# facebookresearch/FlowDec

Measured on AMD Instinct MI355X. Metric: 48 kHz audio-seconds/sec (RTF) for FlowDec-75m @ 6 ODE steps, higher is better.
Workload: dtype bf16; 1 GPU; flowdec_75m enhance(): global batch=8 x 2 s clips @48 kHz (8 per GPU), 6-step euler (NFE 6), T_pad=256 frames, inputs resident in HBM, initial noise drawn inside the timed call, output waveforms all-gathered; global_batch=8, nfe=6, parallelism=batch-shard x1, hipgraph=True, conv_algo=auto

## Files before the change

flowdec_amd/csrc/conv_wino4.hip:

```cpp
#include <type_traits>

#include "conv_common.h"

namespace {

using namespace fdconv;

typedef _Float16 f16;
typedef __attribute__((ext_vector_type(2))) _Float16 f16x2;
typedef __attribute__((ext_vector_type(8))) _Float16 f16x8;
typedef unsigned int u32x2 __attribute__((ext_vector_type(2)));
typedef float f32x2 __attribute__((ext_vector_type(2)));

constexpr int cmax(int a, int b) { return a > b ? a : b; }

constexpr int NTH = 512, TH = 16, TW = 16, HH = TH + 2, HW = TW + 2, BN = 256;
constexpr int CK = 16;
constexpr int SLAB = BN * 32;
constexpr int RSLOT = 2048, NRING = 6;
static_assert(18 % NRING == 0, "the two-chunk loop body turns the ring a whole number of times");
constexpr int RING_BYTES = 8 * NRING * RSLOT;
constexpr int VXI = HH * 4 * 32;
constexpr int V_BYTES = 6 * VXI;
constexpr int V_OFF = RING_BYTES;
constexpr int AFF_OFF = V_OFF + 2 * V_BYTES;
constexpr int RAW_OFF = AFF_OFF + AFF_BYTES;
constexpr int RROW = 20;
constexpr int RROW_BYTES = RROW * 64;
constexpr int RAW_PASSES = 3;
constexpr int RAW_BYTES = RAW_PASSES * NTH * 16;
constexpr int MAIN_BYTES = RAW_OFF + RAW_BYTES;
constexpr int X_BYTES = 8 * 8192;
constexpr int S_PITCH = 128 * 4 + 16;
constexpr int S_BYTES = 128 * S_PITCH;
constexpr int SK_OFF = S_BYTES, SK_BYTES = 4 * NTH * 16;
constexpr int SCK = 2, SCD = 3;
constexpr int WS_BYTES = SCK * SLAB;
constexpr int XS_OFF = SCD * WS_BYTES, XS_BYTES = SCK * 8192;
constexpr int BIAS_OFF = 2 * S_BYTES;
static_assert(BIAS_OFF >= 2 * X_BYTES && BIAS_OFF >= SK_OFF + 2 * SK_BYTES && XS_OFF + SCD * XS_BYTES <= 160 * 1024, "epilogue LDS map");
constexpr int ISC_OFF = BIAS_OFF + 1024;
constexpr int STAT_OFF = ISC_OFF + 1024;
constexpr int LDS_BYTES = cmax(MAIN_BYTES, STAT_OFF + 16384);
constexpr int NPIECE = HH * RROW * 4;
static_assert(LDS_BYTES <= 160 * 1024 && NPIECE <= RAW_PASSES * NTH && AFF_BYTES <= 4 * 1024 && RAW_OFF % 128 == 0, "LDS layout");
constexpr int raw_slot(int c) { return c < 16 ? c + (c >> 2) : (c == 16 ? 14 : 19); }
constexpr int raw_flip(int c) { return c < 16 ? (c >> 3) & 1 : 0; }
constexpr int U_EXP = 9;
constexpr float RAW_MAX = 6000.f;

__device__ __forceinline__ unsigned pack_f16(float a, float b) {
  f16x2 r = {(f16)a, (f16)b};
  return __builtin_bit_cast(unsigned, r);
}
__device__ __forceinline__ f16x2 h2(unsigned u) { return __builtin_bit_cast(f16x2, u); }
__device__ __forceinline__ unsigned u2(f16x2 v) { return __builtin_bit_cast(unsigned, v); }

__device__ __forceinline__ void glds16s(const void* sbase, unsigned voff, unsigned lds_dst) {
  asm volatile("s_mov_b32 m0, %2\n\ts_nop 0\n\tglobal_load_lds_dwordx4 %0, %1" ::"v"(voff), "s"(sbase), "s"(lds_dst) : "memory");
}
__device__ __forceinline__ void glds16s_x2(const void* sbase, unsigned voff, unsigned lds_dst) {
  asm volatile("s_mov_b32 m0, %2\n\ts_nop 0\n\tglobal_load_lds_dwordx4 %0, %1\n\tglobal_load_lds_dwordx4 %0, %1 offset:1024" ::"v"(voff), "s"(sbase), "s"(lds_dst)
               : "memory");
}

template <bool ACT, bool SKIP, bool SC>
__global__ __launch_bounds__(NTH, 2) void conv_wino4_kernel(ConvArgs p) {
  static_assert(!(SKIP && SC), "residual input and folded shortcut exclude each other in this kernel");
  extern __shared__ __attribute__((aligned(16))) char smem[];
  FD_T2(const unsigned long long t2_entry = __builtin_amdgcn_s_memtime();)

  const int bid = blockIdx.x, nblk = gridDim.x;
  int lid;
  {
    const int xcd = bid & 7, qq = nblk >> 3, rr = nblk & 7;
    lid = (xcd < rr ? xcd * (qq + 1) : rr * (qq + 1) + (xcd - rr) * qq) + (bid >> 3);
  }
  if (p.reversed) lid = nblk - 1 - lid;
  int pt = lid;
  const int tw_i = pt % p.tiles_w; pt /= p.tiles_w;
  const int th_i = pt % p.tiles_h;
  const int b = pt / p.tiles_h;
  const int h0 = th_i * TH, w0 = tw_i * TW;
  const int H = p.H, W = p.W;

  const int t = threadIdx.x;
  const int lane = t & 63;
  const int wave = __builtin_amdgcn_readfirstlane(t >> 6);
  const int cq = wave & 3, xt = wave >> 2;

  auto opaque = [&](int v) { asm volatile("" : "+v"(v)); return v; };
  const size_t img_elems = (size_t)H * W;
  const int hb = h0 > 0 ? h0 - 1 : 0;
  const size_t band_pix = (size_t)b * img_elems + (size_t)hb * W;
  const bf16* const sb0 = reinterpret_cast<const bf16*>(p.seg[0].src) + band_pix * p.seg[0].C;
  const bool two3 = p.nseg > 1 && p.seg[1].taps == 9;
  const bf16* const sb1 = two3 ? reinterpret_cast<const bf16*>(p.seg[1].src) + band_pix * p.seg[1].C : sb0;
  const int sC0 = p.seg[0].C, sC1 = two3 ? p.seg[1].C : 0;
  const int nch0 = sC0 / CK, n3 = nch0 + sC1 / CK;
  int hpix[RAW_PASSES];
#pragma unroll
  for (int i = 0; i < RAW_PASSES; ++i) {
    const int sl = t + i * NTH;
    const int slot = sl >> 2;
    const int hr = slot / RROW, ps = slot - hr * RROW;
    const int hc = (ps == 4 || ps == 9 || hr >= HH) ? -1 : ps == 14 ? 16 : ps == 19 ? 17 : ps - ps / 5;
    const int gh = h0 - 1 + hr, gw = w0 - 1 + hc;
    const bool ok = hc >= 0 && gh >= 0 && gh < H && gw >= 0 && gw < W;
    hpix[i] = ((ok ? (gh - hb) * W + gw : 0) << 2) | ((sl & 3) ^ (ok ? 2 * raw_flip(hc) : 0));
  }
  int pA, pB, vbits;
  {
    const int hrow = t >> 5, wt = (t >> 3) & 3, word = t & 7;
    auto raw_at = [&](int c) { return hrow * RROW_BYTES + raw_slot(c) * 64 + raw_flip(c) * 32 + word * 4; };
    const int tidx = hrow * 4 + wt;
    const int vrel = tidx * 32 + (((word >> 2) ^ ((tidx >> 3) & 1)) * 16) + (word & 3) * 4;
    pA = raw_at(4 * wt) | (vrel << 16);
    pB = raw_at(4 * wt + 4) | (raw_at(4 * wt + 5) << 16);
    const int gh = h0 - 1 + hrow, ghe = gh + 14;
    vbits = (w0 - 1 + 4 * wt >= 0 ? 1 : 0) | (gh >= 0 && gh < H ? 2 : 0) | (w0 + 4 * wt + 4 < W ? 4 : 0) | (ghe >= 0 && ghe < H ? 8 : 0);
  }
  const bf16* nbase = sb0;
  int nC2 = 0, ncb = 0;
  int cnext = 0;
  auto next_chunk = [&]() {
    if (cnext < n3) {
      const bool first = cnext < nch0;
      const int cch = first ? cnext : cnext - nch0;
      nbase = first ? sb0 : sb1;
      nC2 = (first ? sC0 : sC1) * 2;
      ncb = cch * CK * 2;
    }
    ++cnext;
  };
  const unsigned rawdst = (unsigned)(RAW_OFF + wave * 1024);
  auto load_halo = [&]() {
    const int on = cnext <= n3 ? 1 : 0;
#pragma unroll
    for (int i = 0; i < RAW_PASSES; ++i) {
      const int hp = opaque(hpix[i]);
      glds16s(nbase, (unsigned)(((hp >> 2) * nC2 + ncb + (hp & 3) * 16) * on), rawdst + i * 8192);
    }
  };
  int affa = AFF_OFF + (t & 7) * 16;
  auto load_affine = [&]() {
    if constexpr (ACT) {
      if (wave < AFF_BYTES / 1024) {
        const int o = opaque(t) * 16;
        glds16s(p.affine + (size_t)b * p.affC * 2, (unsigned)(o < n3 * CK * 8 ? o : 0), (unsigned)(AFF_OFF + wave * 1024));
      }
    }
  };

  auto produce = [&](const bool extra, const int e, const int vbuf, const int affo) {
    const int pa = opaque(pA), pb = opaque(pB), vbt = opaque(vbits);
    const char* const rp = smem + RAW_OFF + (extra ? 14 * RROW_BYTES : 0);
    const int a0 = (pa & 0xffff) ^ (e << 5), a4 = (pb & 0xffff) ^ (e << 5), a5 = (int)((unsigned)pb >> 16) ^ (e << 5);
    const int vrel = (int)((unsigned)pa >> 16);
    char* const vb = smem + V_OFF + vbuf * V_BYTES + (extra ? (vrel ^ 16) + 14 * 4 * 32 : vrel);
    unsigned w_[6];
#pragma unroll
    for (int j = 0; j < 4; ++j) w_[j] = *reinterpret_cast<const unsigned*>(rp + a0 + j * 64);
    w_[4] = *reinterpret_cast<const unsigned*>(rp + a4);
    w_[5] = *reinterpret_cast<const unsigned*>(rp + a5);
    f32x4 af = {0.f, 0.f, 0.f, 0.f};
    if constexpr (ACT) af = *reinterpret_cast<const f32x4*>(smem + opaque(affa) + affo);
    const unsigned mrow = (unsigned)((int)((unsigned)vbt << (extra ? 28 : 30)) >> 31);
    const unsigned m0 = mrow & (unsigned)((int)((unsigned)vbt << 31) >> 31), m5 = mrow & (unsigned)((int)((unsigned)vbt << 29) >> 31);
#pragma unroll
    for (int j = 0; j < 6; ++j) {
      const unsigned u = w_[j];
      const float x0 = __builtin_bit_cast(float, u << 16), x1 = __builtin_bit_cast(float, u & 0xffff0000u);
      unsigned r;
      if constexpr (ACT) {
        const f16x2 zc = {(f16)RAW_MAX, (f16)RAW_MAX};
        r = u2(__builtin_elementwise_min(h2(pack_f16(fd_silu(fmaf(x0, af[0], af[1])), fd_silu(fmaf(x1, af[2], af[3])))), zc));
      } else
        r = pack_f16(__builtin_amdgcn_fmed3f(x0, -RAW_MAX, RAW_MAX), __builtin_amdgcn_fmed3f(x1, -RAW_MAX, RAW_MAX));
      w_[j] = r & (j == 0 ? m0 : j == 5 ? m5 : mrow);
    }
    const f16x2 c4 = {(f16)4.f, (f16)4.f}, cm4 = {(f16)-4.f, (f16)-4.f}, cm5 = {(f16)-5.f, (f16)-5.f}, c2 = {(f16)2.f, (f16)2.f},
                cm2 = {(f16)-2.f, (f16)-2.f};
    const f16x2 z0 = h2(w_[0]), z1 = h2(w_[1]), z2 = h2(w_[2]), z3 = h2(w_[3]), z4 = h2(w_[4]), z5 = h2(w_[5]);
    const f16x2 t1 = __builtin_elementwise_fma(z2, cm4, z4);
    const f16x2 t2 = __builtin_elementwise_fma(z1, cm4, z3);
    const f16x2 t3 = z4 - z2, t4 = z3 - z1;
    *reinterpret_cast<unsigned*>(vb + 0 * VXI) = u2(__builtin_elementwise_fma(z0, c4, __builtin_elementwise_fma(z2, cm5, z4)));
    *reinterpret_cast<unsigned*>(vb + 1 * VXI) = u2(t1 + t2);
    *reinterpret_cast<unsigned*>(vb + 2 * VXI) = u2(t1 - t2);
    *reinterpret_cast<unsigned*>(vb + 4 * VXI) = u2(__builtin_elementwise_fma(t4, c2, t3));
    *reinterpret_cast<unsigned*>(vb + 5 * VXI) = u2(__builtin_elementwise_fma(t4, cm2, t3));
    *reinterpret_cast<unsigned*>(vb + 3 * VXI) = u2(__builtin_elementwise_fma(z1, c4, __builtin_elementwise_fma(z3, cm5, z5)));
  };
  const bool extra_wave = wave == 1;

  const char* wp = reinterpret_cast<const char*>(p.w) + (size_t)xt * 9 * SLAB + cq * 2048;
  asm volatile("" : "+s"(wp));
  const unsigned lane16 = (unsigned)(lane * 16);
  const unsigned wring = (unsigned)(wave * NRING * RSLOT);
  auto dma_step = [&](int f, int slot) {
    glds16s_x2(wp + (f / 9) * 18 * SLAB + (f % 9) * SLAB, lane16, wring + slot * RSLOT);
  };

  const int l31 = lane & 31, lh = lane >> 5;
  const int wa_lane = (int)wring + l31 * 32 + ((lh ^ ((l31 >> 3) & 1)) * 16);
  const int vb0 = V_OFF + xt * 3 * VXI  + l31 * 32 + ((lh ^ ((l31 >> 3) & 1)) * 16);
  const int vb1 = (vb0 ^ ((l31 & 4) << 2)) + 128;

  f32x16 acc[3][2][2];
#pragma unroll
  for (int x = 0; x < 3; ++x)
#pragma unroll
    for (int ct = 0; ct < 2; ++ct)
#pragma unroll
      for (int nt = 0; nt < 2; ++nt)
#pragma unroll
        for (int e = 0; e < 16; ++e) acc[x][ct][nt][e] = 0.f;

  auto lds_wait = [&]() { asm volatile("s_waitcnt lgkmcnt(0)" ::: "memory"); };
  auto barrier = [&]() {
    __builtin_amdgcn_s_barrier();
    asm volatile("" ::: "memory");
  };

  u32x4 qa[3], qb[3];
  auto mma = [&](int xl, int ct, int nt, const u32x4& a, const u32x4& bq) {
    acc[xl][ct][nt] = __builtin_amdgcn_mfma_f32_32x32x16_f16(__builtin_bit_cast(f16x8, a), __builtin_bit_cast(f16x8, bq), acc[xl][ct][nt], 0, 0, 0);
  };
  auto rd = [&](int off) { return *reinterpret_cast<const u32x4*>(smem + off); };
  auto a_off = [&](int k18, int ct) { return wa_lane + (k18 % NRING) * RSLOT + ct * 1024; };
  auto b_off = [&](int k18, int nt) {
    const int s = k18 % 9, half = (k18 / 9) & 1;
    const int dy = s % 3;
    return (dy == 0 ? vb0 : dy == 1 ? vb1 : (vb0 ^ 16) + 256) + half * V_BYTES + (s / 3) * VXI + nt * 1024;
  };

  next_chunk();
  load_halo();
  load_affine();
#pragma unroll
  for (int k = 0; k < NRING; ++k) dma_step(k, k);
  asm volatile("s_waitcnt vmcnt(0)" ::: "memory");
  barrier();
  produce(false, 0, 0, 0);
  if (extra_wave) produce(true, 0, 0, 0);
  next_chunk();
  lds_wait();
  barrier();
  FD_T2(const unsigned long long t2_first = __builtin_amdgcn_s_memtime();)
  qa[0] = rd(a_off(0, 0)); qb[0] = rd(b_off(0, 0)); qb[1] = rd(b_off(0, 1)); qa[1] = rd(a_off(0, 1));

  constexpr int NW = 2 * (NRING - 2);
  for (int c = 0; c < n3; c += 2) {
    int xg = xt;
    asm volatile("" : "+s"(xg));
#pragma clang loop unroll(full)
    for (int k = 0; k < 18; ++k) {
      const int s = k % 9, half = k / 9;
      const int vn = half ^ 1;
      const int xl = s / 3;
      u32x4 &A0 = qa[(2 * k) % 3], &A1 = qa[(2 * k + 1) % 3], &A2 = qa[(2 * k + 2) % 3];
      u32x4 &B0 = qb[(2 * k) % 3], &B1 = qb[(2 * k + 1) % 3], &B2 = qb[(2 * k + 2) % 3];
      if (s >= 4 && s <= 7 && half == 0) asm volatile("s_waitcnt vmcnt(%0)" ::"n"(NW + RAW_PASSES) : "memory");
      else asm volatile("s_waitcnt vmcnt(%0)" ::"n"(NW) : "memory");
      if (s == 8 || (s == 3 && half == 0)) { lds_wait(); barrier(); }
      A2 = rd(a_off(k + 1, 0));
      B2 = rd(b_off(k + 1, 0));
      __builtin_amdgcn_sched_barrier(0);
      mma(xl, 0, 0, A0, B0);
      mma(xl, 0, 1, A0, B1);
      __builtin_amdgcn_sched_barrier(0);
      A0 = rd(a_off(k + 1, 1));
      mma(xl, 1, 0, A1, B0);
      __builtin_amdgcn_sched_barrier(0);
      B0 = rd(b_off(k + 1, 1));
      if (s == 3) { next_chunk(); if (half == 0) load_halo(); }
      dma_step(k + NRING, k % NRING);
      mma(xl, 1, 1, A1, B1);
      __builtin_amdgcn_sched_barrier(0);
      if (s == 0) { if (xg == 0) produce(false, half ^ 1, vn, 128 * (1 + half)); }
      if (s == 1) { if (xg == 1) produce(false, half ^ 1, vn, 128 * (1 + half)); }
      if (s == 2) { if (extra_wave) produce(true, half ^ 1, vn, 128 * (1 + half)); }
      __builtin_amdgcn_sched_barrier(0);
    }
    wp += 36 * SLAB;
    asm volatile("" : "+s"(wp));
    affa += 2 * CK * 8;
  }
  asm volatile("s_waitcnt vmcnt(0)" ::: "memory");
  __syncthreads();
  FD_T2(const unsigned long long t2_loop = __builtin_amdgcn_s_memtime();)

  const size_t row0_pix = (size_t)b * img_elems + (size_t)h0 * W;
  bf16* const out = reinterpret_cast<bf16*>(p.out) + row0_pix * p.Cout;
  const bf16* const skip = SKIP ? reinterpret_cast<const bf16*>(p.skip) + row0_pix * p.Cout : nullptr;
  float* const biast = reinterpret_cast<float*>(smem + BIAS_OFF);
  float* const statt = reinterpret_cast<float*>(smem + STAT_OFF);
  float* const isct = reinterpret_cast<float*>(smem + ISC_OFF);
  auto load_bias_table = [&]() {
    if (t < BN) {
      biast[t] = p.bias ? p.bias[(size_t)(p.bias_rows > 1 ? b : 0) * p.Cout + t] * p.scale : 0.f;
      isct[t] = p.w_scale[t] * p.scale;
    }
  };
  if constexpr (!SC) load_bias_table();
  auto out_off = [&](int tt, int ct, int nt, int ps) {
    const int oct = tt & 15, pp = tt >> 4;
    const int rh = nt * 8 + (pp >> 2), gw = w0 + 4 * (pp & 3) + ps;
    return (rh * W + gw) * p.Cout + ct * 128 + oct * 8;
  };
  auto skip_dma = [&](int r) {
    if constexpr (SKIP) {
      const int tt = opaque(t);
#pragma unroll
      for (int ps = 0; ps < 4; ++ps)
        glds16s(skip, (unsigned)(out_off(tt, r >> 1, r & 1, ps) * 2), (unsigned)(SK_OFF + (r & 1) * SK_BYTES + ps * NTH * 16 + wave * 1024));
    }
  };
  skip_dma(0);
  skip_dma(1);
  FD_T2(
  unsigned long long t2_r[5] = {0, 0, 0, 0, 0};
  t2_r[0] = __builtin_amdgcn_s_memtime();
  )

  const float ka = xt ? 0.f : 1.f, ks = xt ? 4.f : 1.f, kb = xt ? 1.f : 0.f, kd = xt ? 8.f : 1.f, kq = xt ? 0.25f : 1.f;
  auto e1_round = [&](int rd_, int xoff) {
    const int ct = rd_ >> 1, nt = rd_ & 1;
    f32x16 &m0 = acc[0][ct][nt], &m1 = acc[1][ct][nt], &m2 = acc[2][ct][nt];
    const f32x2 kd2 = {kd, kd}, kq2 = {kq, kq}, ka2 = {ka, ka}, ks2 = {ks, ks}, kb2 = {kb, kb};
    char* const xmine = smem + xoff + wave * 8192 + lane * 16;
    const char* const xpeer = smem + xoff + (wave ^ 4) * 8192 + lane * 16;
#pragma unroll
    for (int g = 0; g < 4; ++g) {
      f32x2 snd[2];
#pragma unroll
      for (int h = 0; h < 2; ++h) {
        const int e = 4 * g + 2 * h;
        const f32x2 a1 = {m1[e], m1[e + 1]}, a2 = {m2[e], m2[e + 1]};
        const f32x2 s_ = a1 + a2, d_ = (a1 - a2) * kd2;
        m2[e] = s_[0]; m2[e + 1] = s_[1];
        m1[e] = d_[0]; m1[e + 1] = d_[1];
        snd[h] = d_ * kq2;
      }
      *reinterpret_cast<f32x4*>(xmine + g * 1024) = f32x4{m2[4 * g], m2[4 * g + 1], m2[4 * g + 2], m2[4 * g + 3]};
      *reinterpret_cast<f32x4*>(xmine + 4096 + g * 1024) = f32x4{snd[0][0], snd[0][1], snd[1][0], snd[1][1]};
    }
    lds_wait();
    barrier();
#pragma unroll
    for (int g = 0; g < 4; ++g) {
      const f32x4 r0 = *reinterpret_cast<const f32x4*>(xpeer + g * 1024), r1 = *reinterpret_cast<const f32x4*>(xpeer + 4096 + g * 1024);
#pragma unroll
      for (int h = 0; h < 2; ++h) {
        const int e = 4 * g + 2 * h;
        const f32x2 mm = {m0[e], m0[e + 1]}, ss = {m2[e], m2[e + 1]}, dd = {m1[e], m1[e + 1]};
        const f32x2 q0 = {r0[2 * h], r0[2 * h + 1]}, q1 = {r1[2 * h], r1[2 * h + 1]};
        const f32x2 ya = __builtin_elementwise_fma(ka2, mm, __builtin_elementwise_fma(ks2, ss, q0));
        const f32x2 yb = __builtin_elementwise_fma(kb2, mm, dd + q1);
        m0[e] = ya[0]; m0[e + 1] = ya[1];
        m1[e] = yb[0]; m1[e + 1] = yb[1];
      }
    }
  };
  float ssum[8], ssq[8];
  auto e3_round = [&](int rd_, int soff) {
    const int ct = rd_ >> 1, nt = rd_ & 1;
    f32x16 &m0 = acc[0][ct][nt], &m1 = acc[1][ct][nt];
    char* const sbuf = smem + soff;
    if (nt == 0) {
#pragma unroll
      for (int j = 0; j < 8; ++j) ssum[j] = ssq[j] = 0.f;
    }
    {
      char* const sbase = sbuf + ((2 * xt) * 32 + l31) * S_PITCH + (cq * 32 + 4 * lh) * 4;
#pragma unroll
      for (int g = 0; g < 4; ++g) {
        *reinterpret_cast<f32x4*>(sbase + g * 32) = f32x4{m0[4 * g], m0[4 * g + 1], m0[4 * g + 2], m0[4 * g + 3]};
        *reinterpret_cast<f32x4*>(sbase + 32 * S_PITCH + g * 32) = f32x4{m1[4 * g], m1[4 * g + 1], m1[4 * g + 2], m1[4 * g + 3]};
      }
    }
    lds_wait();
    barrier();
    __builtin_amdgcn_sched_barrier(0);
    if constexpr (SKIP) {
      if (rd_ == 0 || rd_ == 3) asm volatile("s_waitcnt vmcnt(4)" ::: "memory");
      else asm volatile("s_waitcnt vmcnt(8)" ::: "memory");
    }
    {
      const int tt = opaque(t);
      const int oct = tt & 15, pp = tt >> 4;
      const f32x4 bA = *reinterpret_cast<const f32x4*>(biast + ct * 128 + oct * 8), bB = *reinterpret_cast<const f32x4*>(biast + ct * 128 + oct * 8 + 4);
      const float bv[8] = {bA[0], bA[1], bA[2], bA[3], bB[0], bB[1], bB[2], bB[3]};
      const f32x4 iA = *reinterpret_cast<const f32x4*>(isct + ct * 128 + oct * 8), iB = *reinterpret_cast<const f32x4*>(isct + ct * 128 + oct * 8 + 4);
      const float iv[8] = {iA[0], iA[1], iA[2], iA[3], iB[0], iB[1], iB[2], iB[3]};
#pragma unroll
      for (int bt = 0; bt < 2; ++bt) {
        u32x4 packed[2];
        int ooff[2];
#pragma unroll
        for (int q = 0; q < 2; ++q) {
          const int ps = 2 * bt + q;
          ooff[q] = out_off(tt, ct, nt, ps);
          const float* sp = reinterpret_cast<const float*>(sbuf + (pp + ps * 32) * S_PITCH) + oct * 8;
          const f32x4 v0 = *reinterpret_cast<const f32x4*>(sp), v1 = *reinterpret_cast<const f32x4*>(sp + 4);
          float v[8] = {v0[0], v0[1], v0[2], v0[3], v1[0], v1[1], v1[2], v1[3]};
          if constexpr (SKIP) {
            const u32x4 skr = *reinterpret_cast<const u32x4*>(smem + SK_OFF + (rd_ & 1) * SK_BYTES + (ps * NTH + tt) * 16);
            const bf16x8 sk = __builtin_bit_cast(bf16x8, skr);
#pragma unroll
            for (int k = 0; k < 4; ++k) {
              const f32x2 s2_ = {(float)sk[2 * k], (float)sk[2 * k + 1]}, sc2 = {p.scale, p.scale}, b2 = {bv[2 * k], bv[2 * k + 1]};
              const f32x2 i2 = {iv[2 * k], iv[2 * k + 1]}, x_ = {v[2 * k], v[2 * k + 1]};
              const f32x2 r_ = __builtin_elementwise_fma(x_, i2, __builtin_elementwise_fma(s2_, sc2, b2));
              v[2 * k] = r_[0]; v[2 * k + 1] = r_[1];
            }
          }
#pragma unroll
          for (int k = 0; k < 4; ++k) {
#pragma clang fp contract(off)
            f32x2 x = {v[2 * k], v[2 * k + 1]};
            f32x2 s1 = {ssum[2 * k], ssum[2 * k + 1]}, s2 = {ssq[2 * k], ssq[2 * k + 1]};
            if constexpr (!SKIP) {
              const f32x2 b2 = {bv[2 * k], bv[2 * k + 1]}, i2 = {iv[2 * k], iv[2 * k + 1]};
              x = __builtin_elementwise_fma(x, i2, b2);
            }
            s1 += x;
            s2 = __builtin_elementwise_fma(x, x, s2);
            v[2 * k] = x[0]; v[2 * k + 1] = x[1];
            ssum[2 * k] = s1[0]; ssum[2 * k + 1] = s1[1];
            ssq[2 * k] = s2[0]; ssq[2 * k + 1] = s2[1];
          }
          bf16x8 tv;
#pragma unroll
          for (int j = 0; j < 8; ++j) tv[j] = (bf16)v[j];
          packed[q] = __builtin_bit_cast(u32x4, tv);
        }
#pragma unroll
        for (int q = 0; q < 2; ++q) *reinterpret_cast<u32x4*>(out + ooff[q]) = packed[q];
      }
    }
    if (nt == 1 && p.stats) {
#pragma unroll
      for (int j = 0; j < 8; ++j) {
        ssum[j] += __shfl_xor(ssum[j], 16, 64); ssq[j] += __shfl_xor(ssq[j], 16, 64);
        ssum[j] += __shfl_xor(ssum[j], 32, 64); ssq[j] += __shfl_xor(ssq[j], 32, 64);
      }
      if (lane < 16) {
        float* rec = statt + ((ct * 8 + wave) * 16 + lane) * 16;
#pragma unroll
        for (int j = 0; j < 4; ++j) *reinterpret_cast<f32x4*>(rec + 4 * j) = f32x4{ssum[2 * j], ssq[2 * j], ssum[2 * j + 1], ssq[2 * j + 1]};
      }
    }
  };

  if constexpr (SC) {
#pragma unroll
    for (int rd_ = 0; rd_ < 4; ++rd_) {
      e1_round(rd_, (rd_ & 1) * X_BYTES);
      __builtin_amdgcn_sched_barrier(0);
    }
    lds_wait();
    barrier();
    FD_T2(t2_r[1] = __builtin_amdgcn_s_memtime();)
    {
      const int nsc = p.nseg - (sC1 ? 2 : 1);
      const Seg q0 = p.seg[p.nseg - nsc], q1 = p.seg[p.nseg - 1];
      const int S0 = q0.C, Stot = S0 + (nsc > 1 ? q1.C : 0);
      const int nstage = Stot / (16 * SCK);
      const bf16* const xb0 = reinterpret_cast<const bf16*>(q0.src) + row0_pix * q0.C;
      const bf16* const xb1 = reinterpret_cast<const bf16*>(q1.src) + row0_pix * q1.C;
      const char* const wsc = reinterpret_cast<const char*>(p.w) + (size_t)(n3 + 1) * 18 * SLAB + cq * 2048;
      static_assert(SCK == 2, "a stage row = 2 K steps x 2 halves x 16 B; K step kk of the weights is loaded by wave group xt = kk");
      int xsrc[2];
#pragma unroll
      for (int i = 0; i < 2; ++i) {
        const int r = ((i * 8 + wave) * 64 + lane) >> 2;
        const int xtile = r & 63, xj = r >> 6;
        const int piece = (lane & 3) ^ ((r >> 2) & 3);
        xsrc[i] = (((xtile >> 2) * W + w0 + 4 * (xtile & 3) + xj) << 8) | (piece * 16);
      }
      const unsigned lane16e = (unsigned)(lane * 16);
      auto stage_dma = [&](int st, int slot) {
        const int ste = st < nstage ? st : 0;
        const int c0 = ste * 16 * SCK;
        const bool first = c0 < S0;
        const bf16* const xb = first ? xb0 : xb1;
        const int Cs = first ? S0 : Stot - S0, cc = first ? c0 : c0 - S0;
#pragma unroll
        for (int i = 0; i < 2; ++i)
          glds16s(xb, (unsigned)(((xsrc[i] >> 8) * Cs + cc) * 2 + (xsrc[i] & 255)), (unsigned)(XS_OFF + slot * XS_BYTES + i * 8192 + wave * 1024));
        glds16s_x2(wsc + (size_t)(ste * SCK + xt) * SLAB, lane16e, (unsigned)(slot * WS_BYTES + xt * SLAB + cq * 2048));
      };
      const int wa_sc = cq * 2048 + l31 * 32 + ((lh ^ ((l31 >> 3) & 1)) * 16);
      const int xb_row = XS_OFF + ((2 * xt) * 64 + l31) * 64;
      const int xb_sw = (l31 >> 2) & 3;
#pragma unroll
      for (int d = 0; d < SCD - 1; ++d) stage_dma(d, d);
      int slot = 0;
      for (int st = 0; st < nstage; ++st) {
        asm volatile("s_waitcnt vmcnt(%0)" ::"n"(4 * (SCD - 2)) : "memory");
        lds_wait();
        barrier();
        const int nslot = slot == 0 ? SCD - 1 : slot - 1;
        stage_dma(st + SCD - 1, nslot);
        const int wo = slot * WS_BYTES, xo = slot * XS_BYTES;
        u32x4 af[SCK][2], bq[SCK][2][2];
#pragma unroll
        for (int kk = 0; kk < SCK; ++kk) {
          af[kk][0] = rd(wa_sc + wo + kk * SLAB);
          af[kk][1] = rd(wa_sc + wo + kk * SLAB + 1024);
#pragma unroll
          for (int pl = 0; pl < 2; ++pl)
#pragma unroll
            for (int nt = 0; nt < 2; ++nt) bq[kk][pl][nt] = rd(xb_row + xo + (pl * 64 + nt * 32) * 64 + (((kk * 2 + lh) ^ xb_sw) * 16));
        }
        __builtin_amdgcn_sched_barrier(0);
#pragma unroll
        for (int kk = 0; kk < SCK; ++kk)
#pragma unroll
          for (int pl = 0; pl < 2; ++pl)
#pragma unroll
            for (int nt = 0; nt < 2; ++nt) {
              acc[pl][0][nt] = __builtin_amdgcn_mfma_f32_32x32x16_bf16(__builtin_bit_cast(bf16x8, af[kk][0]), __builtin_bit_cast(bf16x8, bq[kk][pl][nt]), acc[pl][0][nt], 0, 0, 0);
              acc[pl][1][nt] = __builtin_amdgcn_mfma_f32_32x32x16_bf16(__builtin_bit_cast(bf16x8, af[kk][1]), __builtin_bit_cast(bf16x8, bq[kk][pl][nt]), acc[pl][1][nt], 0, 0, 0);
            }
        __builtin_amdgcn_sched_barrier(0);
        slot = slot + 1 == SCD ? 0 : slot + 1;
      }
      asm volatile("s_waitcnt vmcnt(0)" ::: "memory");
      lds_wait();
      barrier();
      load_bias_table();
    }
    FD_T2(t2_r[2] = __builtin_amdgcn_s_memtime();)
#pragma unroll
    for (int rd_ = 0; rd_ < 4; ++rd_) {
      e3_round(rd_, (rd_ & 1) * S_BYTES);
      __builtin_amdgcn_sched_barrier(0);
    }
  } else {
#pragma unroll
    for (int rd_ = 0; rd_ < 4; ++rd_) {
      e1_round(rd_, 0);
      if constexpr (SKIP) { lds_wait(); barrier(); }
      e3_round(rd_, SKIP ? 0 : X_BYTES);
      if constexpr (SKIP) {
        lds_wait();
        barrier();
        if (rd_ < 2) skip_dma(rd_ + 2);
      }
      __builtin_amdgcn_sched_barrier(0);
    }
  }
  FD_T2(t2_r[3] = __builtin_amdgcn_s_memtime();)
  if (p.stats) {
    lds_wait();
    barrier();
    const int ch = t >> 1, which = t & 1;
    const int ct = ch >> 7, oc = (ch >> 3) & 15, j = ch & 7;
    const float* src = statt + (ct * 8 * 16 + oc) * 16 + 2 * j + which;
    float a = 0.f;
#pragma unroll
    for (int w_ = 0; w_ < 8; ++w_) a += src[w_ * 256];
    const int tile = th_i * p.tiles_w + tw_i;
    p.stats[((size_t)b * p.tiles_h * p.tiles_w + tile) * p.CoutPad * 2 + t] = a;
  }
  FD_T2(
  if (p.dbg && t == 0 && bid < 8192) {
    const unsigned long long t2_end = __builtin_amdgcn_s_memtime();
    unsigned long long* d = p.dbg + (size_t)bid * 8;
    d[0] = t2_first - t2_entry; d[1] = t2_loop - t2_first; d[2] = t2_end - t2_loop;
    d[3] = t2_r[1] - t2_r[0]; d[4] = t2_r[2] - t2_r[1]; d[5] = t2_r[3] - t2_r[2]; d[6] = t2_end - t2_r[3]; d[7] = t2_r[0] - t2_loop;
  }
  )
}

__device__ __forceinline__ float wino4_u(const float* g, int xi) {
  const float g0 = g[0], g1 = g[1], g2 = g[2];
  switch (xi) {
    case 0: return 0.25f * g0;
    case 1: return -(g0 + g1 + g2) / 6.f;
    case 2: return (-g0 + g1 - g2) / 6.f;
    case 3: return g0 / 24.f + g1 / 12.f + g2 / 6.f;
    case 4: return g0 / 24.f - g1 / 12.f + g2 / 6.f;
    default: return g2;
  }
}

constexpr int SC_EXP_MAX = 60;
__global__ void wino4_scale_kernel(const float* __restrict__ w, const float* __restrict__ w_sc, float* __restrict__ tab, int Cout, int Cin, int S) {
  __shared__ float red[256], red_sc[256];
  const int co = blockIdx.x, t = threadIdx.x;
  float m = 0.f, msc = 0.f;
  if (co < Cout) {
    for (int i = t; i < Cin * 3; i += 256) {
      const float* g = w + ((size_t)co * Cin * 3 + i) * 3;
#pragma unroll
      for (int xi = 0; xi < 6; ++xi) m = fmaxf(m, fabsf(wino4_u(g, xi)));
    }
    if (w_sc)
      for (int i = t; i < S; i += 256) msc = fmaxf(msc, fabsf(w_sc[(size_t)co * S + i]));
  }
  red[t] = m;
  red_sc[t] = msc;
  __syncthreads();
  for (int o = 128; o > 0; o >>= 1) {
    if (t < o) { red[t] = fmaxf(red[t], red[t + o]); red_sc[t] = fmaxf(red_sc[t], red_sc[t + o]); }
    __syncthreads();
  }
  if (t == 0) {
    int k = 0;
    m = red[0];
    msc = red_sc[0];
    if (m > 0.f && m < 3.0e38f) {
      int e;
      frexpf(m, &e);
      k = U_EXP - e;
      k = k < -100 ? -100 : (k > 100 ? 100 : k);
      if (msc > 0.f && msc < 3.0e38f) {
        int es;
        frexpf(msc, &es);
        if (k > SC_EXP_MAX - es) k = SC_EXP_MAX - es;
      }
    }
    tab[co] = ldexpf(1.f, -k);
    tab[BN + co] = ldexpf(1.f, k);
  }
}

__global__ void wino4_pack_kernel(const float* __restrict__ w, f16* __restrict__ dst, const float* __restrict__ tab, int Cout, int C0, int C1) {
  const int Cin = C0 + C1, nchunks = Cin / CK;
  const long long total = (long long)nchunks * 18 * BN * CK;
  for (long long i = blockIdx.x * (long long)blockDim.x + threadIdx.x; i < total; i += (long long)gridDim.x * blockDim.x) {
    const int k = (int)(i % CK);
    long long r = i / CK;
    const int n = (int)(r % BN); r /= BN;
    const int dy = (int)(r % 3); r /= 3;
    const int slot = (int)(r % 6);
    const int xi = slot < 3 ? slot : (slot == 3 ? 5 : slot - 1);
    const int chunk = (int)(r / 6);
    const int c = chunk * CK + k;
    const int co = ((n >> 5) & 1) * 128 + (n >> 6) * 32 + (n & 31);
    float v = 0.f;
    if (co < Cout) v = wino4_u(w + (((size_t)co * Cin + c) * 3 + dy) * 3, xi) * tab[BN + co];
    const int half = (k >> 3) ^ ((n >> 3) & 1);
    dst[(i - k) + half * 8 + (k & 7)] = (f16)v;
  }
}

__global__ void wino4_pack_sc_kernel(const float* __restrict__ w, bf16* __restrict__ dst, const float* __restrict__ tab, int Cout, int S) {
  const long long total = (long long)(S / CK) * BN * CK;
  for (long long i = blockIdx.x * (long long)blockDim.x + threadIdx.x; i < total; i += (long long)gridDim.x * blockDim.x) {
    const int k = (int)(i % CK);
    long long r = i / CK;
    const int n = (int)(r % BN);
    const int ks = (int)(r / BN);
    const int co = ((n >> 5) & 1) * 128 + (n >> 6) * 32 + (n & 31);
    const float v = co < Cout ? w[(size_t)co * S + ks * CK + k] * tab[BN + co] : 0.f;
    const int half = (k >> 3) ^ ((n >> 3) & 1);
    dst[(i - k) + half * 8 + (k & 7)] = (bf16)v;
  }
}

}

bool fd_wino4_supported(int Cout, int C0, int C1, int S0, int S1, int ksize) {
  return ksize == 3 && Cout == BN && C0 > 0 && C0 % 32 == 0 && C1 % 32 == 0 && S0 % 32 == 0 && S1 % 32 == 0 && (S1 == 0 || S0 > 0) &&
         (C0 + C1) * 8 <= AFF_BYTES;
}
bool fd_wino4_shape_ok(int H, int W) { return H % TH == 0 && W % TW == 0; }

namespace {
constexpr long long W4_HDR = 4096;
}

long long fd_wino4_packed_bytes(int Cout, int C0, int C1, int S0, int S1) {
  (void)Cout;
  return W4_HDR + (long long)((C0 + C1) / CK + 1) * 18 * SLAB + (long long)((S0 + S1) / CK) * SLAB + 16 * 1024;
}

int fd_wino4_pack_weights(const float* w, const float* w_sc, void* packed, int Cout, int C0, int C1, int S0, int S1, hipStream_t st) {
  const long long total = (long long)((C0 + C1) / CK) * 18 * BN * CK;
  const int blocks = (int)((total + 255) / 256 > 4096 ? 4096 : (total + 255) / 256);
  float* const tab = reinterpret_cast<float*>(packed);
  char* const steps = reinterpret_cast<char*>(packed) + W4_HDR;
  hipLaunchKernelGGL(wino4_scale_kernel, dim3(BN), dim3(256), 0, st, w, w_sc, tab, Cout, C0 + C1, w_sc ? S0 + S1 : 0);
  hipLaunchKernelGGL(wino4_pack_kernel, dim3(blocks), dim3(256), 0, st, w, (f16*)steps, tab, Cout, C0, C1);
  if (w_sc) {
    const long long tsc = (long long)((S0 + S1) / CK) * BN * CK;
    const int bsc = (int)((tsc + 255) / 256 > 4096 ? 4096 : (tsc + 255) / 256);
    hipLaunchKernelGGL(wino4_pack_sc_kernel, dim3(bsc), dim3(256), 0, st, w_sc,
                       reinterpret_cast<bf16*>(steps + (size_t)((C0 + C1) / CK + 1) * 18 * SLAB), tab, Cout, S0 + S1);
  }
  FD_LAUNCH_CHECK();
  return FD_OK;
}

namespace {
template <bool ACT>
int set_attr4() {
  FD_HIP(hipFuncSetAttribute(reinterpret_cast<const void*>(conv_wino4_kernel<ACT, false, false>), hipFuncAttributeMaxDynamicSharedMemorySize, LDS_BYTES));
  FD_HIP(hipFuncSetAttribute(reinterpret_cast<const void*>(conv_wino4_kernel<ACT, true, false>), hipFuncAttributeMaxDynamicSharedMemorySize, LDS_BYTES));
  FD_HIP(hipFuncSetAttribute(reinterpret_cast<const void*>(conv_wino4_kernel<ACT, false, true>), hipFuncAttributeMaxDynamicSharedMemorySize, LDS_BYTES));
  return FD_OK;
}
template <bool ACT>
void launch4(const ConvArgs& a, bool sc, dim3 grid, dim3 block, hipStream_t st) {
  if (sc) hipLaunchKernelGGL((conv_wino4_kernel<ACT, false, true>), grid, block, LDS_BYTES, st, a);
  else if (a.skip) hipLaunchKernelGGL((conv_wino4_kernel<ACT, true, false>), grid, block, LDS_BYTES, st, a);
  else hipLaunchKernelGGL((conv_wino4_kernel<ACT, false, false>), grid, block, LDS_BYTES, st, a);
}
}

int fd_wino4_init_attributes() {
  FD_TRY(set_attr4<false>());
  FD_TRY(set_attr4<true>());
  return FD_OK;
}

int fd_wino4_launch(ConvArgs a, hipStream_t st) {
  FD_REQUIRE(fd_wino4_shape_ok(a.H, a.W), "fd_conv2d: FD_WINOGRAD4 needs H %% 16 == 0 and W %% 16 == 0 (got %d x %d)", a.H, a.W);
  bool sc = false;
  for (int s = 0; s < a.nseg; ++s) sc = sc || a.seg[s].taps == 1;
  a.w_scale = reinterpret_cast<const float*>(a.w);
  a.w = reinterpret_cast<const char*>(a.w) + W4_HDR;
  FD_REQUIRE(!(sc && a.skip), "fd_conv2d: FD_WINOGRAD4 takes a folded shortcut or a residual input, not both");
  a.tiles_h = a.H / TH;
  a.tiles_w = a.W / TW;
  a.tiles_n = 1;
  a.CoutPad = BN;
  const long long nblk = (long long)a.B * a.tiles_h * a.tiles_w;
  FD_REQUIRE(nblk > 0 && nblk < (1ll << 31), "conv grid out of range");
  const dim3 grid((unsigned)nblk), block(NTH);
  if (a.affine) launch4<true>(a, sc, grid, block, st);
  else launch4<false>(a, sc, grid, block, st);
  FD_LAUNCH_CHECK();
  return FD_OK;
}
```

Measured before the change: 131.7 audio-seconds/second.

## Remap Winograd input-transform work so all waves share halo columns via DPP

```diff
diff --git a/flowdec_amd/csrc/conv_wino4.hip b/flowdec_amd/csrc/conv_wino4.hip
--- a/flowdec_amd/csrc/conv_wino4.hip
+++ b/flowdec_amd/csrc/conv_wino4.hip
@@ -1,6 +1,7 @@
 #include <type_traits>
 
 #include "conv_common.h"
+#include "wino4_layout.h"
 
 namespace {
 
@@ -14,21 +15,18 @@
 
 constexpr int cmax(int a, int b) { return a > b ? a : b; }
 
-constexpr int NTH = 512, TH = 16, TW = 16, HH = TH + 2, HW = TW + 2, BN = 256;
+using fdw4::NTH, fdw4::HH, fdw4::HW, fdw4::RROW, fdw4::RROW_BYTES, fdw4::RAW_PASSES, fdw4::RAW_BYTES, fdw4::NPIECE, fdw4::VXI;
+constexpr int TH = 16, TW = 16, BN = 256;
+static_assert(HH == TH + 2 && HW == TW + 2, "wino4_layout.h describes this tile");
 constexpr int CK = 16;
 constexpr int SLAB = BN * 32;
 constexpr int RSLOT = 2048, NRING = 6;
 static_assert(18 % NRING == 0, "the two-chunk loop body turns the ring a whole number of times");
 constexpr int RING_BYTES = 8 * NRING * RSLOT;
-constexpr int VXI = HH * 4 * 32;
 constexpr int V_BYTES = 6 * VXI;
 constexpr int V_OFF = RING_BYTES;
 constexpr int AFF_OFF = V_OFF + 2 * V_BYTES;
 constexpr int RAW_OFF = AFF_OFF + AFF_BYTES;
-constexpr int RROW = 20;
-constexpr int RROW_BYTES = RROW * 64;
-constexpr int RAW_PASSES = 3;
-constexpr int RAW_BYTES = RAW_PASSES * NTH * 16;
 constexpr int MAIN_BYTES = RAW_OFF + RAW_BYTES;
 constexpr int X_BYTES = 8 * 8192;
 constexpr int S_PITCH = 128 * 4 + 16;
@@ -42,10 +40,7 @@
 constexpr int ISC_OFF = BIAS_OFF + 1024;
 constexpr int STAT_OFF = ISC_OFF + 1024;
 constexpr int LDS_BYTES = cmax(MAIN_BYTES, STAT_OFF + 16384);
-constexpr int NPIECE = HH * RROW * 4;
 static_assert(LDS_BYTES <= 160 * 1024 && NPIECE <= RAW_PASSES * NTH && AFF_BYTES <= 4 * 1024 && RAW_OFF % 128 == 0, "LDS layout");
-constexpr int raw_slot(int c) { return c < 16 ? c + (c >> 2) : (c == 16 ? 14 : 19); }
-constexpr int raw_flip(int c) { return c < 16 ? (c >> 3) & 1 : 0; }
 constexpr int U_EXP = 9;
 constexpr float RAW_MAX = 6000.f;
 
@@ -101,24 +96,19 @@
   int hpix[RAW_PASSES];
 #pragma unroll
   for (int i = 0; i < RAW_PASSES; ++i) {
-    const int sl = t + i * NTH;
-    const int slot = sl >> 2;
-    const int hr = slot / RROW, ps = slot - hr * RROW;
-    const int hc = (ps == 4 || ps == 9 || hr >= HH) ? -1 : ps == 14 ? 16 : ps == 19 ? 17 : ps - ps / 5;
-    const int gh = h0 - 1 + hr, gw = w0 - 1 + hc;
-    const bool ok = hc >= 0 && gh >= 0 && gh < H && gw >= 0 && gw < W;
-    hpix[i] = ((ok ? (gh - hb) * W + gw : 0) << 2) | ((sl & 3) ^ (ok ? 2 * raw_flip(hc) : 0));
-  }
-  int pA, pB, vbits;
+    const fdw4::Req rq = fdw4::raw_request(t + i * NTH);
+    const int gh = h0 - 1 + rq.row, gw = w0 - 1 + rq.col;
+    const bool ok = rq.col >= 0 && gh >= 0 && gh < H && gw >= 0 && gw < W;
+    hpix[i] = ((ok ? (gh - hb) * W + gw : 0) << 2) | (ok ? rq.piece : t & 3);
+  }
+  int pA, vbits, pword;
   {
-    const int hrow = t >> 5, wt = (t >> 3) & 3, word = t & 7;
-    auto raw_at = [&](int c) { return hrow * RROW_BYTES + raw_slot(c) * 64 + raw_flip(c) * 32 + word * 4; };
-    const int tidx = hrow * 4 + wt;
-    const int vrel = tidx * 32 + (((word >> 2) ^ ((tidx >> 3) & 1)) * 16) + (word & 3) * 4;
-    pA = raw_at(4 * wt) | (vrel << 16);
-    pB = raw_at(4 * wt + 4) | (raw_at(4 * wt + 5) << 16);
-    const int gh = h0 - 1 + hrow, ghe = gh + 14;
-    vbits = (w0 - 1 + 4 * wt >= 0 ? 1 : 0) | (gh >= 0 && gh < H ? 2 : 0) | (w0 + 4 * wt + 4 < W ? 4 : 0) | (ghe >= 0 && ghe < H ? 8 : 0);
+    const fdw4::Item it = fdw4::item(t);
+    pA = fdw4::raw_addr(it.row, 6 * it.k, 0, it.word) | (fdw4::v_addr(it.row, fdw4::first_tile(it.k), it.word) << 16);
+    const int gh = h0 - 1 + it.row;
+    vbits = (it.k != 0 || w0 > 0 ? 1 : 0) | (gh >= 0 && gh < H ? 2 : 0) | (it.k != 2 || w0 + TW < W ? 4 : 0) | (it.active ? 8 : 0) |
+            (it.active && it.k == 1 ? 16 : 0);
+    pword = it.word;
   }
   const bf16* nbase = sb0;
   int nC2 = 0, ncb = 0;
@@ -142,7 +132,7 @@
       glds16s(nbase, (unsigned)(((hp >> 2) * nC2 + ncb + (hp & 3) * 16) * on), rawdst + i * 8192);
     }
   };
-  int affa = AFF_OFF + (t & 7) * 16;
+  int affa = AFF_OFF + pword * 16;
   auto load_affine = [&]() {
     if constexpr (ACT) {
       if (wave < AFF_BYTES / 1024) {
@@ -152,20 +142,16 @@
     }
   };
 
-  auto produce = [&](const bool extra, const int e, const int vbuf, const int affo) {
-    const int pa = opaque(pA), pb = opaque(pB), vbt = opaque(vbits);
-    const char* const rp = smem + RAW_OFF + (extra ? 14 * RROW_BYTES : 0);
-    const int a0 = (pa & 0xffff) ^ (e << 5), a4 = (pb & 0xffff) ^ (e << 5), a5 = (int)((unsigned)pb >> 16) ^ (e << 5);
-    const int vrel = (int)((unsigned)pa >> 16);
-    char* const vb = smem + V_OFF + vbuf * V_BYTES + (extra ? (vrel ^ 16) + 14 * 4 * 32 : vrel);
+  auto produce = [&](const int e, const int vbuf, const int affo) {
+    const int pa = opaque(pA), vbt = opaque(vbits);
+    const char* const rp = smem + RAW_OFF + ((pa & 0xffff) ^ (e << 5));
+    char* const vb = smem + V_OFF + vbuf * V_BYTES + (int)((unsigned)pa >> 16);
     unsigned w_[6];
 #pragma unroll
-    for (int j = 0; j < 4; ++j) w_[j] = *reinterpret_cast<const unsigned*>(rp + a0 + j * 64);
-    w_[4] = *reinterpret_cast<const unsigned*>(rp + a4);
-    w_[5] = *reinterpret_cast<const unsigned*>(rp + a5);
+    for (int j = 0; j < 6; ++j) w_[j] = *reinterpret_cast<const unsigned*>(rp + j * 64);
     f32x4 af = {0.f, 0.f, 0.f, 0.f};
     if constexpr (ACT) af = *reinterpret_cast<const f32x4*>(smem + opaque(affa) + affo);
-    const unsigned mrow = (unsigned)((int)((unsigned)vbt << (extra ? 28 : 30)) >> 31);
+    const unsigned mrow = (unsigned)((int)((unsigned)vbt << 30) >> 31);
     const unsigned m0 = mrow & (unsigned)((int)((unsigned)vbt << 31) >> 31), m5 = mrow & (unsigned)((int)((unsigned)vbt << 29) >> 31);
 #pragma unroll
     for (int j = 0; j < 6; ++j) {
@@ -179,20 +165,29 @@
         r = pack_f16(__builtin_amdgcn_fmed3f(x0, -RAW_MAX, RAW_MAX), __builtin_amdgcn_fmed3f(x1, -RAW_MAX, RAW_MAX));
       w_[j] = r & (j == 0 ? m0 : j == 5 ? m5 : mrow);
     }
+    const unsigned l4 = (unsigned)__builtin_amdgcn_update_dpp(0, (int)w_[4], 0x111, 0xf, 0xf, true);
+    const unsigned l5 = (unsigned)__builtin_amdgcn_update_dpp(0, (int)w_[5], 0x111, 0xf, 0xf, true);
+    const unsigned r0 = (unsigned)__builtin_amdgcn_update_dpp(0, (int)w_[0], 0x101, 0xf, 0xf, true);
+    const unsigned r1 = (unsigned)__builtin_amdgcn_update_dpp(0, (int)w_[1], 0x101, 0xf, 0xf, true);
+    const bool mid = (vbt & 16) != 0;
     const f16x2 c4 = {(f16)4.f, (f16)4.f}, cm4 = {(f16)-4.f, (f16)-4.f}, cm5 = {(f16)-5.f, (f16)-5.f}, c2 = {(f16)2.f, (f16)2.f},
                 cm2 = {(f16)-2.f, (f16)-2.f};
-    const f16x2 z0 = h2(w_[0]), z1 = h2(w_[1]), z2 = h2(w_[2]), z3 = h2(w_[3]), z4 = h2(w_[4]), z5 = h2(w_[5]);
-    const f16x2 t1 = __builtin_elementwise_fma(z2, cm4, z4);
-    const f16x2 t2 = __builtin_elementwise_fma(z1, cm4, z3);
-    const f16x2 t3 = z4 - z2, t4 = z3 - z1;
-    *reinterpret_cast<unsigned*>(vb + 0 * VXI) = u2(__builtin_elementwise_fma(z0, c4, __builtin_elementwise_fma(z2, cm5, z4)));
-    *reinterpret_cast<unsigned*>(vb + 1 * VXI) = u2(t1 + t2);
-    *reinterpret_cast<unsigned*>(vb + 2 * VXI) = u2(t1 - t2);
-    *reinterpret_cast<unsigned*>(vb + 4 * VXI) = u2(__builtin_elementwise_fma(t4, c2, t3));
-    *reinterpret_cast<unsigned*>(vb + 5 * VXI) = u2(__builtin_elementwise_fma(t4, cm2, t3));
-    *reinterpret_cast<unsigned*>(vb + 3 * VXI) = u2(__builtin_elementwise_fma(z1, c4, __builtin_elementwise_fma(z3, cm5, z5)));
-  };
-  const bool extra_wave = wave == 1;
+    auto transform = [&](char* const v, const unsigned d0, const unsigned d1, const unsigned d2, const unsigned d3, const unsigned d4, const unsigned d5) {
+      const f16x2 z0 = h2(d0), z1 = h2(d1), z2 = h2(d2), z3 = h2(d3), z4 = h2(d4), z5 = h2(d5);
+      const f16x2 t1 = __builtin_elementwise_fma(z2, cm4, z4);
+      const f16x2 t2 = __builtin_elementwise_fma(z1, cm4, z3);
+      const f16x2 t3 = z4 - z2, t4 = z3 - z1;
+      *reinterpret_cast<unsigned*>(v + 0 * VXI) = u2(__builtin_elementwise_fma(z0, c4, __builtin_elementwise_fma(z2, cm5, z4)));
+      *reinterpret_cast<unsigned*>(v + 1 * VXI) = u2(t1 + t2);
+      *reinterpret_cast<unsigned*>(v + 2 * VXI) = u2(t1 - t2);
+      *reinterpret_cast<unsigned*>(v + 4 * VXI) = u2(__builtin_elementwise_fma(t4, c2, t3));
+      *reinterpret_cast<unsigned*>(v + 5 * VXI) = u2(__builtin_elementwise_fma(t4, cm2, t3));
+      *reinterpret_cast<unsigned*>(v + 3 * VXI) = u2(__builtin_elementwise_fma(z1, c4, __builtin_elementwise_fma(z3, cm5, z5)));
+    };
+    if (vbt & 8)
+      transform(vb, mid ? l4 : w_[0], mid ? l5 : w_[1], mid ? w_[0] : w_[2], mid ? w_[1] : w_[3], mid ? w_[2] : w_[4], mid ? w_[3] : w_[5]);
+    if (mid) transform(vb + 32, w_[2], w_[3], w_[4], w_[5], r0, r1);
+  };
 
   const char* wp = reinterpret_cast<const char*>(p.w) + (size_t)xt * 9 * SLAB + cq * 2048;
   asm volatile("" : "+s"(wp));
@@ -242,8 +237,7 @@
   for (int k = 0; k < NRING; ++k) dma_step(k, k);
   asm volatile("s_waitcnt vmcnt(0)" ::: "memory");
   barrier();
-  produce(false, 0, 0, 0);
-  if (extra_wave) produce(true, 0, 0, 0);
+  produce(0, 0, 0);
   next_chunk();
   lds_wait();
   barrier();
@@ -278,9 +272,8 @@
       dma_step(k + NRING, k % NRING);
       mma(xl, 1, 1, A1, B1);
       __builtin_amdgcn_sched_barrier(0);
-      if (s == 0) { if (xg == 0) produce(false, half ^ 1, vn, 128 * (1 + half)); }
-      if (s == 1) { if (xg == 1) produce(false, half ^ 1, vn, 128 * (1 + half)); }
-      if (s == 2) { if (extra_wave) produce(true, half ^ 1, vn, 128 * (1 + half)); }
+      if (s == 0) { if (xg == 0) produce(half ^ 1, vn, 128 * (1 + half)); }
+      if (s == 1) { if (xg == 1) produce(half ^ 1, vn, 128 * (1 + half)); }
       __builtin_amdgcn_sched_barrier(0);
     }
     wp += 36 * SLAB;
diff --git a/flowdec_amd/csrc/wino4_layout.h b/flowdec_amd/csrc/wino4_layout.h
--- /dev/null
+++ b/flowdec_amd/csrc/wino4_layout.h
@@ -0,0 +1,44 @@
+#pragma once
+
+namespace fdw4 {
+
+constexpr int NTH = 512;
+constexpr int HH = 18, HW = 18;
+constexpr int RROW = 20;
+constexpr int RROW_BYTES = RROW * 64;
+constexpr int RAW_PASSES = 3;
+constexpr int RAW_BYTES = RAW_PASSES * NTH * 16;
+constexpr int NPIECE = HH * RROW * 4;
+constexpr int VXI = HH * 4 * 32;
+static_assert(NPIECE <= RAW_PASSES * NTH && RROW_BYTES % 128 == 0, "RAW layout");
+
+constexpr int raw_slot(int c) { return c + c / 6; }
+constexpr int raw_flip(int c) { return c >= 12 ? 1 : 0; }
+constexpr int raw_col(int ps) { return (ps == 6 || ps == 13) ? -1 : ps - ps / 7; }
+
+struct Req { int row, col, piece; };
+constexpr Req raw_request(int sl) {
+  const int slot = sl >> 2, hr = slot / RROW, ps = slot - hr * RROW;
+  const int hc = hr >= HH ? -1 : raw_col(ps);
+  return {hr, hc, (sl & 3) ^ (hc >= 0 ? 2 * raw_flip(hc) : 0)};
+}
+constexpr int raw_addr(int row, int c, int e, int word) { return row * RROW_BYTES + raw_slot(c) * 64 + ((raw_flip(c) ^ e) * 32) + word * 4; }
+
+struct Item { bool active; int row, word, k; };
+constexpr Item item(int t) {
+  const int lane = t & 63, wave = t >> 6, l16 = lane & 15, gq = l16 / 3;
+  const int g = (lane >> 4) * 5 + gq, k = l16 - 3 * gq;
+  if (l16 == 15 || g >= 18) return {false, 2 * wave + (lane >> 5), 0, 0};
+  if (g < 8) return {true, 2 * wave, g, k};
+  if (g >= 10) return {true, 2 * wave + 1, g - 10, k};
+  const int left = 2 * wave + (g - 8);
+  return {true, 16 + (left >> 3), left & 7, k};
+}
+constexpr int v_addr(int row, int tile, int word) {
+  const int tidx = row * 4 + tile;
+  return tidx * 32 + (((word >> 2) ^ ((tidx >> 3) & 1)) * 16) + (word & 3) * 4;
+}
+constexpr int first_tile(int k) { return k == 2 ? 3 : k; }
+static_assert(v_addr(5, 2, 6) == v_addr(5, 1, 6) + 32 && v_addr(17, 2, 1) == v_addr(17, 1, 1) + 32, "tile 2 follows tile 1 in the same swizzle phase");
+
+}
```

Result: faster. 133.0 audio-seconds/second, median of 6 (+1.0%).
